# ACCtools/alignasm

Measured on AMD Instinct MI355X. Metric: contigs_per_sec, higher is better.
Workload: dtype int64

## Files before the change

### alignasm_amd/csrc/aasm_kernels.h

```cpp
#pragma once
#include <cstddef>
#include "aasm_dev.h"
#include "../../include/alignasm_amd.h"

namespace aasm {

struct PqK;
struct WS {
    int64_t C, R, R0, S, VT, ET;
    int32_t K, nsl;
    int32_t avg_sidetracks;
    int32_t xcd_map;
    int32_t mw_compact;
    int32_t sort_depth_test;
    const int64_t *rec_off, *in_qs, *in_qe, *in_rs, *in_re, *in_qt, *in_rng_off, *rql, *rqr, *rrl;
    const int32_t *in_chr;
    const uint8_t *in_fwd, *in_mq;
    const char *cs_text;
    const int64_t *cs_off;
    int64_t *rng_rec;
    int64_t rng_stride;
    int32_t *cs_bad;
    int32_t *perm, *dupflag, *np, *pstart;
    int64_t *s_qs, *s_qe, *s_rs, *s_re, *s_qt, *s_rb;
// ... 3047 lines not shown
}

#if defined(AASM_HOST_EMUL)
static int64_t g_k9_stat[64];
#define K9STAT(i, n) (g_k9_stat[i] += (n))
#else
#define K9STAT(i, n) do {} while (0)
#endif
struct SelCtx {
    const WS *w;
    int64_t c, b, N, V, vb, cap;
    int32_t src, dest;
    int32_t *pathA, *pathB, *pathT, *pre2, *stamp;
    Dist *dist2;
    OutElem *cur;
    int64_t *cls;
    int32_t epoch, last_head, last_pos;
    int32_t res_ppos;
    int32_t *out_dst;
    int32_t out_n, out_flushed;
    int32_t pa_base, pa_n;
    int32_t wu, wv, wpv, wvf;
    int32_t cw_pa, cw_n;
    bool err, res_lds;
    int lane;
    char *lds;
    int64_t n_ispr_e, n_ispr_v, n_path_e, n_out_e;
#if defined(AASM_KPROF) && !defined(AASM_HOST_EMUL)
    int64_t kp_t0, kp_acc[8];
#endif
};
#if defined(AASM_KPROF) && !defined(AASM_HOST_EMUL)
#define SPROF(s, i) do { __builtin_amdgcn_s_waitcnt(0); const int64_t t1_ = (int64_t)__builtin_amdgcn_s_memtime(); __builtin_amdgcn_s_waitcnt(0); (s).kp_acc[i] += t1_ - (s).kp_t0; (s).kp_t0 = t1_; } while (0)
#else
#define SPROF(s, i) do {} while (0)
#endif

#define ISPR_MAX_E 192
#define SEL_WIN 64
struct SelLds {
    int32_t pb_buf[2 * SEL_WIN];
    int64_t wq[ISPR_MAX_E];
    int32_t wr[ISPR_MAX_E];
    int8_t tgt[ISPR_MAX_E];
    uint8_t fl[ISPR_MAX_E];
    Dist dist[64];
    int32_t excl[64], u[64], vj[64];
    int8_t pre[64];
    uint8_t reach[64];
    int32_t res[2 * 64];
};
#define AASM_SEL_LDS_BYTES 6656
#define AASM_SELREC_LDS_BYTES 512
static_assert(sizeof(SelLds) <= AASM_SEL_LDS_BYTES, "LDS budget");
static_assert(offsetof(SelLds, wq) == AASM_SELREC_LDS_BYTES, "kb_sel_recover allocates the write buffer alone");
#define ISPR_WIDE 127
struct SelWide { Dist dist[ISPR_WIDE + 1]; int32_t excl[ISPR_WIDE + 2]; int32_t vj[ISPR_WIDE + 1]; uint8_t pre[ISPR_WIDE + 1]; uint8_t reach[ISPR_WIDE + 1]; };
static_assert(offsetof(SelLds, wq) + sizeof(SelWide) <= offsetof(SelLds, res), "the wide DP state must end before the result array");

AASM_DEV void sel_out_flush(SelCtx &s) {
    SelLds *L = (SelLds *)s.lds;
    wave_lds_sync();
    const int32_t n = s.out_n - s.out_flushed;
    for (int32_t t = s.lane; t < 2 * n; t += AASM_WAVE) s.out_dst[2 * s.out_flushed + t] = L->pb_buf[t];
    s.out_flushed = s.out_n;
    wave_lds_sync();
}
AASM_DEV void sel_out_begin(SelCtx &s, int32_t *dst) { s.out_dst = dst; s.out_n = 0; s.out_flushed = 0; }
AASM_DEV void sel_push(SelCtx &s, int32_t u, int32_t v, int32_t pos_v) {
    SelLds *L = (SelLds *)s.lds;
    if (s.out_n >= s.cap) { s.err = true; return; }
    const int32_t slot = s.out_n - s.out_flushed;
    if (s.lane == 0) { L->pb_buf[2 * slot] = u; L->pb_buf[2 * slot + 1] = v; }
    s.out_n++;
    s.last_head = v; s.last_pos = pos_v;
    if (s.out_n - s.out_flushed == SEL_WIN) sel_out_flush(s);
}
#if !defined(AASM_HOST_EMUL)
AASM_DEV void sel_push_lanes(SelCtx &s, int32_t l0, int32_t m, int32_t u, int32_t v) {
    SelLds *L = (SelLds *)s.lds;
    if (s.out_n + m > s.cap) { s.err = true; return; }
    const int32_t slot0 = s.out_n - s.out_flushed, room = SEL_WIN - slot0;
    const int32_t first = m < room ? m : room;
    const int32_t k = s.lane - l0;
    if (k >= 0 && k < first) { L->pb_buf[2 * (slot0 + k)] = u; L->pb_buf[2 * (slot0 + k) + 1] = v; }
    s.out_n += first;
    if (s.out_n - s.out_flushed == SEL_WIN) sel_out_flush(s);
    if (m > first) {
        if (k >= first && k < m) { L->pb_buf[2 * (k - first)] = u; L->pb_buf[2 * (k - first) + 1] = v; }
        s.out_n += m - first;
    }
}
#endif

AASM_DEV int32_t sel_recover(SelCtx &s, int32_t kidx) {
    const WS &w = *s.w;
    const int64_t K = w.K;
    if (kidx < 0 || kidx >= w.kfound[s.c]) return 0;
    const I4 *kcand = w.kcand + 2 * s.c * (3 * K + 1);
    const HNode *nodes = heap_arena(w, s.c);
    int32_t ns = 0;
    int32_t cur = w.klast[s.c * K + kidx];
    while (cur != -1) {
        if (ns >= s.cap) { s.err = true; return -1; }
        const I4 cd = kcand[2 * (int64_t)cur];
        const HNode nd = nodes[cd.x];
        if (s.lane == 0) { s.pathT[2 * ns] = nd.u; s.pathT[2 * ns + 1] = nd.v; }
        ns++;
        cur = cd.y;
    }
    wave_fence();
    sel_out_begin(s, s.pathA);
    int32_t idx = ns - 1, cv = s.src;
    int32_t st_u = -1, st_v = -1;
    if (idx >= 0) { st_u = uni(s.pathT[2 * idx]); st_v = uni(s.pathT[2 * idx + 1]); }
    while (cv != s.dest || idx >= 0) {
        if (s.err) return -1;
        if (idx >= 0 && cv == st_u) {
            sel_push(s, cv, st_v, -1);
            cv = st_v; idx--;
            if (idx >= 0) { st_u = uni(s.pathT[2 * idx]); st_v = uni(s.pathT[2 * idx + 1]); }
        } else {
            const int32_t *rec = w.tnx16 + 16 * (s.vb + cv);
#if defined(AASM_HOST_EMUL)
            for (int t = 0; t < 16; t++) {
                const int32_t nx = rec[t];
                if (nx < 0) { s.err = true; return -1; }
                sel_push(s, cv, nx, -1);
                cv = nx;
                if (s.err || cv == s.dest || (idx >= 0 && cv == st_u)) break;
            }
#else
            const bool in = s.lane < 16;
            const int32_t x = in ? rec[s.lane] : -1;
            const uint64_t stop = wave_ballot(in && (x == s.dest || (idx >= 0 && x == st_u)));
            const uint64_t bad = wave_ballot(in && x < 0);
            const int32_t m = stop ? ffs64(stop) : 16;
            if (bad && ffs64(bad) <= m) { s.err = true; return -1; }
            int32_t from = wave_shfl_up(x, 1, cv);
            if (s.lane == 0) from = cv;
            sel_push_lanes(s, 0, m, from, x);
            cv = wave_bcast(x, m - 1);
#endif
        }
    }
    if (s.err) return -1;
    sel_out_flush(s);
    return s.out_n;
}

#define SETTLE_SCAN_MAX 48
AASM_DEV void sel_classify_edge(const WS &w, int64_t vb, int32_t dest, const int32_t *pathA, int32_t la, int32_t t, int32_t *mark, int32_t ord, int64_t *cls) {
    const int32_t tu = pathA[2 * t], hv = pathA[2 * t + 1];
    const int32_t nvv = (t + 1 < la) ? pathA[2 * t + 3] : -1;
    const int32_t a = w.v_i[vb + hv], b = w.v_j[vb + hv];
    const int32_t pu = w.fwd_pos[vb + tu], pv = w.fwd_pos[vb + hv];
    const int32_t pnv = nvv >= 0 ? w.fwd_pos[vb + nvv] : -1;
    if (hv != dest) {
        atomic_min_i32(&mark[a], ord);
        if (b != a) atomic_min_i32(&mark[b], ord);
    }
    int32_t fl = (a == b) ? 1 : 0;
    const int32_t dpos = pnv - pu;
    if (nvv >= 0 && (dpos == 2 || dpos == 3)) {
        const int64_t *tp = w.tp_ptr + vb + pu;
        const int64_t p0 = tp[0], p1 = tp[1], p2 = tp[2], p3 = (dpos == 3) ? tp[3] : p2;
        if (p3 - p0 <= SETTLE_SCAN_MAX) {
            const bool y_first = pv == pu + 2;
            const int32_t py = y_first ? pu + 1 : pu + 2;
            bool u_nv = false, u_y = false, y_nv = false, y_v = false, v_y = false;
            for (int64_t e = p0; e < p3; e++) {
                const int32_t tg = w.te_pk[e].x;
                const int32_t row = e < p1 ? 0 : e < p2 ? 1 : 2;
                if (row == 0) { u_nv |= tg == pnv; u_y |= tg == py; }
// ... 549 lines not shown
                    const int64_t up = (dd.qry + dd.ref) - (mind.qry + mind.ref), down = (int64_t)mind.anom - dd.anom;
                    int32_t kind = -1;
                    if (ans_idx == -1 || up * ans_down < down * ans_up) { ans_up = up; ans_down = down; ans_idx = i; ans_d = dd; kind = 2; }
                    else if (dist_sel_equal(dd, ans_d)) kind = 3;
                    if (kind >= 0) { if (k.lane == 0) put(n, i, kind); n++; }
                }
            }
        }
    }
    return n;
}
AASM_DEV void kb_sel_plan(const KCtx &k, const WS &w) {
    const int64_t c = k.bid;
    const int32_t n = sel_has_graph(w, c) ? sel_plan_wave(k, w, c, false) : 0;
    if (k.lane == 0) w.nconv[c] = n;
}
AASM_DEV void kb_sel_planfill(const KCtx &k, const WS &w) {
    const int64_t c = k.bid;
    if (!sel_has_graph(w, c)) return;
    const int32_t n = w.nconv[c];
    if (n > SEL_PLAN_KEEP) { sel_plan_wave(k, w, c, true); return; }
    const int32_t N = (int32_t)(w.rec_off[c + 1] - w.rec_off[c]), V = w.ctgV[c];
    const int32_t *keep = w.plan_kk + c * (int64_t)(2 * SEL_PLAN_KEEP);
    const int64_t j0 = w.conv_off[c];
    for (int32_t t = k.lane; t < n; t += AASM_WAVE) {
        const int64_t j = j0 + t;
        w.cv_ctg[j] = (int32_t)c; w.cv_k[j] = keep[2 * t]; w.cv_ord[j] = t; w.cv_kind[j] = keep[2 * t + 1]; w.cv_szr[j] = N + 2; w.cv_szv[j] = V;
    }
}

AASM_DEV void sel_ctx_init(SelCtx &s, const KCtx &k, const WS &w, int64_t c) {
    const int64_t gb = w.rec_off[c];
    s.w = &w; s.c = c; s.b = gb - w.R0; s.N = w.rec_off[c + 1] - gb; s.V = w.ctgV[c]; s.vb = w.voff[c]; s.cap = s.N + 2;
    s.src = (int32_t)(s.V - 2); s.dest = (int32_t)(s.V - 1);
    s.epoch = 0; s.last_head = -1; s.last_pos = -1; s.res_ppos = -1; s.err = false; s.res_lds = false; s.out_dst = nullptr; s.out_n = s.out_flushed = 0;
    s.pa_base = 0; s.pa_n = 0; s.wu = s.wv = s.wpv = s.wvf = 0; s.cls = nullptr;
    s.lane = k.lane; s.lds = k.lds; s.n_ispr_e = s.n_ispr_v = s.n_path_e = s.n_out_e = 0;
    s.cw_pa = -1; s.cw_n = 0;
}
AASM_DEV void sel_flush_counters(const SelCtx &s, const WS &w) {
    if (s.lane == 0) {
        atomic_add(&w.counters[CNT_ISPR_E], s.n_ispr_e); atomic_add(&w.counters[CNT_ISPR_V], s.n_ispr_v);
        atomic_add(&w.counters[CNT_PATH_E], s.n_path_e); atomic_add(&w.counters[CNT_OUT_E], s.n_out_e);
    }
}

AASM_DEV void sel_conv_setup(SelCtx &s, const KCtx &k, const WS &w, int64_t j) {
    sel_ctx_init(s, k, w, w.cv_ctg[j]);
    const int64_t ro = w.cv_roff[j], vo = w.cv_voff[j];
    s.pathA = w.cv_path + 6 * ro; s.pathB = s.pathA + 2 * s.cap; s.pathT = s.pathB + 2 * s.cap;
    s.pre2 = w.cv_pre2 + vo; s.stamp = w.cv_stamp + vo; s.dist2 = w.cv_dist2 + vo;
    s.cur = w.cv_out + ro; s.cls = (int64_t *)s.cur;
}
AASM_DEV void kb_sel_recover(const KCtx &k, const WS &w) {
    const int64_t j = k.bid;
    SelCtx s;
    sel_conv_setup(s, k, w, j);
    const int32_t la = sel_recover(s, w.cv_k[j]);
    if (k.lane == 0) w.cv_la[j] = (la <= 0 || s.err) ? -1 : la;
}
AASM_DEV void kb_sel_classify(const KCtx &k, const WS &w) {
    const int64_t j = k.bid;
    const int32_t la = w.cv_la[j];
    if (la <= 0) return;
    const int64_t c = w.cv_ctg[j], vb = w.voff[c], ro = w.cv_roff[j];
    const int32_t dest = w.ctgV[c] - 1;
    const int64_t cap = (w.rec_off[c + 1] - w.rec_off[c]) + 2;
    (void)cap;
    int32_t *mark = w.mark_time + (w.rec_off[c] - w.R0);
    for (int32_t t = k.tid; t < la; t += k.nthreads) sel_classify_edge(w, vb, dest, w.cv_path + 6 * ro, la, t, mark, w.cv_ord[j], (int64_t *)(w.cv_out + ro));
}
AASM_DEV void kb_sel_convert(const KCtx &k, const WS &w) {
    const int64_t j = k.bid;
    const int64_t c = w.cv_ctg[j];
    SelCtx s;
    sel_conv_setup(s, k, w, j);
#if defined(AASM_KPROF) && !defined(AASM_HOST_EMUL)
    for (int i_ = 0; i_ < 8; i_++) s.kp_acc[i_] = 0;
    __builtin_amdgcn_s_waitcnt(0); s.kp_t0 = (int64_t)__builtin_amdgcn_s_memtime(); __builtin_amdgcn_s_waitcnt(0);
#endif
    int64_t cov = 0;
    int32_t n = 0;
    const int32_t la = w.cv_la[j];
    if (la <= 0) s.err = true;
    else { K9STAT(0, 1); K9STAT(1, la); n = sel_upgrade_emit(s, la, cov); }
    if (k.lane == 0) { w.cv_n[j] = n; w.cv_cov[j] = cov; w.cv_err[j] = s.err ? 1 : 0; }
#if defined(AASM_KPROF) && !defined(AASM_HOST_EMUL)
    if (k.lane == 0 && w.cv_ord[j] == 0) for (int i_ = 0; i_ < 8; i_++) w.prof_sel[c * 8 + i_] = s.kp_acc[i_];
#endif
    (void)c;
    sel_flush_counters(s, w);
}

AASM_DEV void sel_all_append(const KCtx &k, const WS &w, int64_t c, const OutElem *src, int32_t n, const int32_t *mark, int32_t ord) {
    int64_t off = 0, r = 0;
    if (k.lane == 0) { off = (int64_t)atomic_add(&w.counters[CNT_POOL], (int64_t)n); r = (int64_t)atomic_add(&w.counters[CNT_AR], (int64_t)1); }
    off = wave_bcast(off, 0); r = wave_bcast(r, 0);
    if (off + n <= w.pool_cap && r < w.ar_cap) {
        copy_resolved(w.pool + off, src, n, mark, ord, k.lane);
        if (k.lane == 0) { w.ar_ctg[r] = (int32_t)c; w.ar_gen[r] = w.all_gen[c]; w.ar_seq[r] = w.all_seq[c]; w.ar_off[r] = off; w.ar_len[r] = n; }
    } else if (k.lane == 0) {
        atomic_add(&w.counters[CNT_OVF], (int64_t)1);
    }
    if (k.lane == 0) w.all_seq[c] += 1;
    wave_fence();
}

AASM_DEV void kb_sel_final(const KCtx &k, const WS &w) {
    const int64_t c = k.bid;
    const int64_t gb = w.rec_off[c], N = w.rec_off[c + 1] - gb, b = gb - w.R0;
    const bool L0 = (k.lane == 0);
// ... 204 lines not shown
```

### alignasm_amd/csrc/aasm_pipeline.h

```cpp
#pragma once
#include <algorithm>
#include <cstdlib>
#include <cstring>
#include <map>
#include <string>
#include <vector>

#include "../../include/alignasm_amd.h"
#include "aasm_kernels.h"
#include "aasm_enum.h"

namespace aasm {

enum Kern {
#define AASM_PIPELINE_KERNELS(K, KL)                                                                                                  \
    K(KN_CS_RANGES, aasm_k0_cs_ranges, 256, ALL_LANES, kb_cs_ranges)                                                                  \
    KL(KN_SORT, aasm_k1_sort, 256, 1, AASM_SORT_LDS_BYTES, 2, kb_sort)                                                                \
    K(KN_SORT_RANK, aasm_k1_sort_rank, 256, ALL_LANES, kb_sort_rank)                                                                  \
    KL(KN_SORT_FIX, aasm_k1_sort_fix, AASM_WAVE, 1, AASM_SORTFIX_LDS_BYTES, 1, kb_sort_fix)                                           \
    K(KN_GATHER_PARTS, aasm_k1_gather_parts, AASM_WAVE, 1, kb_gather_parts)                                                           \
    K(KN_OV_COUNT, aasm_k2_ov_count, 256, ALL_LANES, kb_ov_count)                                                                     \
    K(KN_OV_MERGE, aasm_k2_ov_merge, 256, ALL_LANES, kb_ov_merge)                                                                     \
    K(KN_VCOUNT, aasm_k2_vcount, 256, ALL_LANES, kb_vcount)                                                                           \
    K(KN_VFILL_REC, aasm_k2_vfill_rec, 256, ALL_LANES, kb_vfill_rec)                                                                  \
    K(KN_VFILL_SLOT, aasm_k2_vfill_slot, 256, ALL_LANES, kb_vfill_slot)                                                               \
    K(KN_NSL, aasm_k4_nsl, 256, ALL_LANES, kb_nsl)                                                                                    \
    K(KN_ROW_COUNT, aasm_k4_row_count, 256, ALL_LANES, kb_row_count)                                                                  \
    K(KN_ROW_FILL, aasm_k4_row_fill, AASM_WAVE, 1, kb_row_fill)                                                                       \
                               \
    KL(KN_GRAPH, aasm_k46_graph, GB_TPB, 1, AASM_GB_LDS_BYTES, 5, kb_graph_build<GB_MAXV, GB_MAXE>)                                   \
                                                     \
    KL(KN_GRAPH_L, aasm_k46_graph_l, GB_TPB, 1, AASM_GB_LDS_BYTES_T(GB_MAXV_L, GB_MAXE_L), 2, kb_graph_build<GB_MAXV_L, GB_MAXE_L>)   \
    K(KN_REV_FILL, aasm_k6_rev_fill, 256, ALL_LANES, kb_rev_fill)                                                                     \
    KL(KN_REV_FILL_W, aasm_k6_rev_fill_w, AASM_WAVE, 1, AASM_REVF_LDS_BYTES, 8, kb_rev_fill_w)                                        \
                    \
    KL(KN_REV_FILL_ORD, aasm_k6_rev_fill_ord, AASM_WAVE, 1, AASM_REVO_LDS_BYTES, 2, kb_rev_fill_ord)                                  \
    KL(KN_REV_FILL_ORD_S, aasm_k6_rev_fill_ord_s, AASM_WAVE, 1, AASM_REVO_LDS_BYTES_V(REV_ORD_MIDV), 6, kb_rev_fill_ord)              \
    KL(KN_SORT_ROWS_REV, aasm_k6_rev_place, AASM_WAVE, 1, AASM_REVP_LDS_BYTES, 4, kb_rev_place)                                       \
    K(KN_REV_HDR, aasm_k6_rev_hdr, 256, ALL_LANES, kb_rev_hdr)                                                                        \
    KL(KN_REV_SWEEP, aasm_k6_rev_sweep, AASM_WAVE, 1, AASM_REV_LDS_BYTES, 8, kb_rev_sweep<AASM_WAVE>)                                 \
    KL(KN_FWD_SWEEP, aasm_k5_fwd_sweep, AASM_WAVE, 1, AASM_FWD_LDS_BYTES, 8, kb_fwd_sweep<AASM_WAVE>)                                 \
    KL(KN_REV_SWEEP_G, aasm_k6_rev_sweep_g, AASM_WAVE, 1, (AASM_WAVE / AASM_SWEEP_G) * AASM_REV_LDS_BYTES, 4, kb_rev_sweep<AASM_SWEEP_G>) \
    KL(KN_FWD_SWEEP_G, aasm_k5_fwd_sweep_g, AASM_WAVE, 1, (AASM_WAVE / AASM_SWEEP_G) * AASM_FWD_LDS_BYTES, 4, kb_fwd_sweep<AASM_SWEEP_G>) \
    K(KN_CHILDREN, aasm_k7_children, 256, ALL_LANES, kb_children)                                                                     \
    K(KN_HEAP_CAP, aasm_k7_heap_cap, 256, ALL_LANES, kb_heap_cap)                                                                     \
    KL(KN_SIDETRACK_W, aasm_k7_sidetrack_w, AASM_WAVE, 1, AASM_SIDE_LDS_BYTES, 8, kb_sidetrack_w)                                     \
    K(KN_HEAP_HDR, aasm_k7_heap_hdr, 256, ALL_LANES, kb_heap_hdr)                                                                     \
    KL(KN_HEAP, aasm_k7_heap, AASM_WAVE, 1, AASM_HEAP_LDS_BYTES, 5, kb_heap<false, HEAP_RING_1W, HEAP_QN_1W>)                         \
    KL(KN_HEAP_MW, aasm_k7_heap_mw, AASM_WAVE * 4, 1, AASM_MW_LDS_BYTES(4), 4, kb_heap_mw)                                            \
    KL(KN_HEAP_MW8, aasm_k7_heap_mw8, AASM_WAVE * 8, 1, AASM_MW_LDS_BYTES(8), 4, kb_heap_mw)                                          \
    KL(KN_HEAP_MW16, aasm_k7_heap_mw16, AASM_WAVE * 16, 1, AASM_MW_LDS_BYTES(16), 4, kb_heap_mw)                                      \
    K(KN_MW_RANK, aasm_k7_mw_rank, 256, ALL_LANES, kb_mw_rank)                                                                        \
                                    \
    KL(KN_ENUM, aasm_k8_enum, AASM_WAVE, 1, AASM_EMUL_OR(AASM_ENUM_LDS_BYTES, AASM_ENUM2_LDS_BYTES), 4,                               \
       AASM_EMUL_OR(kb_enum_heap, kb_enum_lsm<64>))                                                                                   \
    KL(KN_ENUM_S, aasm_k8_enum_s, AASM_WAVE, 1, AASM_EMUL_OR(AASM_ENUM_LDS_BYTES, AASM_ENUM2_LDS_BYTES_F(EQ_FSMALL)), 5,              \
       AASM_EMUL_OR(kb_enum_heap, kb_enum_lsm<EQ_FSMALL>))                                                                            \
    KL(KN_ENUM_HEAP, aasm_k8_enum_heap, AASM_WAVE, 1, AASM_ENUM_LDS_BYTES, 2, kb_enum_heap)                                           \
    KL(KN_SELECT, aasm_k9_select, AASM_WAVE, 1, AASM_SEL_LDS_BYTES, 5, kb_select)                                                     \
    K(KN_GATHER_OUT, aasm_k9_gather_out, AASM_WAVE, 1, kb_gather_out)                                                                 \
    K(KN_TOPO_COUNT, aasm_k9_topo_count, 256, ALL_LANES, kb_topo_count)                                                               \
    K(KN_TOPO_FILL, aasm_k9_topo_fill, AASM_WAVE, 1, kb_topo_fill)                                                                    \
    K(KN_SEL_PLAN, aasm_k9_sel_plan, AASM_WAVE, 1, kb_sel_plan)                                                                       \
    K(KN_SEL_PLANFILL, aasm_k9_sel_planfill, AASM_WAVE, 1, kb_sel_planfill)                                                           \
    KL(KN_SEL_RECOVER, aasm_k9_sel_recover, AASM_WAVE, 1, AASM_SELREC_LDS_BYTES, 8, kb_sel_recover)                                   \
    K(KN_SEL_CLASSIFY, aasm_k9_sel_classify, 256, ALL_LANES, kb_sel_classify)                                                         \
    KL(KN_SEL_CONVERT, aasm_k9_sel_convert, AASM_WAVE, 1, AASM_SEL_LDS_BYTES, 5, kb_sel_convert)                                      \
    K(KN_SEL_FINAL, aasm_k9_sel_final, AASM_WAVE, 1, kb_sel_final)                                                                    \
            \
    KL(KN_CHAIN, aasm_k67_chain, AASM_WAVE * CHAIN_WAVES, CHAIN_WAVES, AASM_CHAIN_LDS_BYTES, 5, kb_chain<true>)                       \
                 \
    KL(KN_CHAIN3, aasm_k67_chain3, AASM_WAVE * (CHAIN_WAVES - 1), CHAIN_WAVES - 1, AASM_CHAIN_LDS_BYTES, 5, kb_chain<false>)          \
    K(KN_K7_PREP, aasm_k7_prep, 256, ALL_LANES, kb_k7_prep)                                                                           \
    K(KN_TNX, aasm_k9_tnx, 256, ALL_LANES, kb_tnx)                                                                                    \
    K(KN_TNX16, aasm_k9_tnx16, 256, ALL_LANES, kb_tnx16)                                                                              \
                                                                  \
    KL(KN_TNX16_WG, aasm_k9_tnx16_wg, TNX_TPB, 1, AASM_TNXWG_LDS_BYTES, 4, kb_tnx16_wg)
    AASM_PIPELINE_KERNELS(AASM_ROW_ID, AASM_ROW_ID)
};
constexpr int kern_block[] = {AASM_PIPELINE_KERNELS(AASM_ROW_BLOCK, AASM_ROW_BLOCK)};

AASM_DEV void run_kernel_body(int kn, const KCtx &k, const WS &w) {
    switch (kn) {
#define K(id, sym, block, lanes, ...) case id: __VA_ARGS__(k, w); break;
#define KL(id, sym, block, lanes, lds, waves, ...) case id: __VA_ARGS__(k, w); break;
        AASM_PIPELINE_KERNELS(K, KL)
#undef K
#undef KL
    }
}

template <class B> void launch(B &be, int kn, int64_t nblocks, const WS &w) { be.launch(kn, nblocks, kern_block[kn], w); }

static inline int64_t cdiv(int64_t a, int64_t b) { return (a + b - 1) / b; }
#ifndef AASM_CHAIN_ORD_MAX
#define AASM_CHAIN_ORD_MAX 1024
#endif
#define AASM_CHAIN_SMALL_BATCH 1536

#ifndef AASM_GROUPED_MIN
#define AASM_GROUPED_MIN 2560
#endif
struct PipelineSizes { int64_t C = 0, R = 0, S = 0, VT = 0, ET = 0, HT = 0, bad_record = -1; };

struct Hooks {
    bool seq_select, enum_heap, enum_small, grid_order, graph_launches, chain_half, launch_failure, wrap_devices, dirty_scan, chain_own_queue;
    int32_t heap_mw, chain, chain_test, root_ring, sort_depth;
    int32_t mw;
    int64_t range_limit;
};
static inline Hooks decode_hooks(const aasm_opts &o) {
    const int32_t h0 = o.reserved[0], h2 = o.reserved[2], ch = h0 & AASM_H0_CHAIN_MASK;
    Hooks h;
    h.seq_select = h0 & AASM_H0_SEQ_SELECT; h.enum_heap = h0 & AASM_H0_ENUM_HEAP; h.enum_small = h0 & AASM_H0_ENUM_SMALL;
    h.grid_order = h0 & AASM_H0_GRID_ORDER; h.graph_launches = h0 & AASM_H0_GRAPH_LAUNCHES; h.chain_half = ch == AASM_H0_CHAIN_HALF;
    h.heap_mw = (h0 & AASM_H0_HEAP_MW_ALL) ? 1 : (h0 & AASM_H0_HEAP_MW_NONE) ? 2 : 0;
    h.chain = ch == AASM_H0_CHAIN_ALL ? 1 : ch == AASM_H0_CHAIN_NONE ? 2 : 0;
    h.mw = (h0 & AASM_H0_MW_MASK) >> AASM_H0_MW_SHIFT; h.range_limit = o.reserved[1];
    h.launch_failure = h2 & AASM_H2_LAUNCH_FAILURE; h.wrap_devices = h2 & AASM_H2_WRAP_DEVICES; h.dirty_scan = h2 & AASM_H2_DIRTY_SCAN;
    h.chain_test = (h2 & AASM_H2_CHAIN_DONE_LOST) ? 2 : (h2 & AASM_H2_CHAIN_HDR_LOST) ? 1 : 0; h.chain_own_queue = h2 & AASM_H2_CHAIN_OWN_QUEUE;
    h.root_ring = (h2 & AASM_H2_SMALL_ROOT_RING) ? 4 : 0; h.sort_depth = (h2 & AASM_H2_SORT_DEPTH_MASK) >> AASM_H2_SORT_DEPTH_SHIFT;
    return h;
}

struct FormSizes { int64_t C, R, K, VT, ET, MAXV, NCHAIN, HTM, NMW, MAXN; };
struct Forms {
    bool grouped, dense, mw_ranked;
    int rev_fill, chain, mw_kern, enum_kern;
};
static inline Forms choose_forms(const FormSizes &s, const Hooks &h, bool host_emulation) {
    Forms f;
    f.dense = s.ET > 6 * s.VT;
    f.grouped = !f.dense && s.C >= AASM_GROUPED_MIN;
    f.rev_fill = f.dense && s.MAXV <= REV_ORD_MAXV ? (s.MAXV <= REV_ORD_MIDV ? KN_REV_FILL_ORD_S : KN_REV_FILL_ORD) : f.dense ? KN_REV_FILL_W : KN_REV_FILL;
    f.chain = !h.chain_own_queue && s.NCHAIN <= AASM_CHAIN_ORD_MAX ? KN_CHAIN : KN_CHAIN3;
    const int mw_waves = (h.mw == 4 || h.mw == 8 || h.mw == 16) ? h.mw : s.NMW * 16 <= 6144 ? 16 : s.NMW * 8 <= 6144 ? 8 : 4;
    f.mw_kern = mw_waves == 16 ? KN_HEAP_MW16 : mw_waves == 8 ? KN_HEAP_MW8 : KN_HEAP_MW;
    f.mw_ranked = h.mw != AASM_H0_MW_INPUT_ORDER && s.NMW >= 2 && s.NMW <= 32768;
    const bool enum_heap = host_emulation || h.enum_heap || s.MAXN > AASM_ENUM_MAX_N;
    f.enum_kern = enum_heap ? KN_ENUM_HEAP : ((s.C > 14 * 256 && s.C <= 20 * 256 && s.K > 21) || h.enum_small) ? KN_ENUM_S : KN_ENUM;
    return f;
}

template <class B>
int run_pipeline(B &be, const aasm_batch_in &in, const aasm_opts &opts, WS &w, PipelineSizes &sz) {
    std::memset(&w, 0, sizeof(w));
    const int64_t C = in.n_contigs;
    int64_t rr[2];
    be.read_i64s({in.ctg_rec_off, in.ctg_rec_off + C}, rr);
    const int64_t R0 = rr[0], R1 = rr[1];
    const int64_t R = R1 - R0;
    w.C = C; w.R = R; w.R0 = R0;
    w.K = opts.max_paths > 0 ? opts.max_paths : 10000;
    w.nsl = opts.non_skip_linkable ? 1 : 0;
    const Hooks h = decode_hooks(opts);
    w.xcd_map = h.grid_order ? 0 : 1; w.sort_depth_test = h.sort_depth;
    w.chain_mode = h.chain; w.chain_test = h.chain_test; w.chain_rn = h.root_ring;
    w.chain_ord = h.chain_own_queue ? 0 : 1;
    w.chain_all = (!h.chain_half && C <= AASM_CHAIN_SMALL_BATCH) ? 1 : 0;
    w.chain_minN = (int32_t)std::min<int64_t>(std::max<int64_t>(2048, 4 * (R / std::max<int64_t>(C, 1))), INT32_MAX);
    if (h.chain_half) w.chain_minN = (int32_t)std::min<int64_t>(std::max<int64_t>(1, cdiv(R, std::max<int64_t>(C, 1))), INT32_MAX);
    w.rec_off = in.ctg_rec_off; w.in_qs = in.qry_str; w.in_qe = in.qry_end; w.in_rs = in.ref_str; w.in_re = in.ref_end;
    w.in_qt = in.qry_total; w.in_chr = in.ref_chr; w.in_fwd = in.aln_fwd; w.in_mq = in.map_qul;
    w.in_rng_off = in.rec_rng_off; w.rql = in.rng_qry_l; w.rqr = in.rng_qry_r; w.rrl = in.rng_ref_l; w.rng_stride = 1;
    sz.C = C; sz.R = R;
    if (C <= 0 || R <= 0) return AASM_E_INVAL;

#define A(field, type, n, name) w.field = (type *)be.alloc(name, sizeof(type) * (size_t)((n) > 0 ? (n) : 1))
#define AZ(field, type, n, name) do { A(field, type, n, name); be.zero_alloc(w.field, sizeof(type) * (size_t)((n) > 0 ? (n) : 1)); } while (0)
#define CHECK_ALLOC() do { if (be.oom()) return AASM_E_NOMEM; if (be.failed()) return AASM_E_HIP; } while (0)

    AZ(status, int32_t, C, "status");
    AZ(prof_heap, int64_t, C * 8, "prof_heap"); AZ(prof_sel, int64_t, C * 8, "prof_sel"); AZ(prof_gb, int64_t, C * 8, "prof_gb");
    AZ(counters, int64_t, CNT_N, "counters");
    AZ(dupflag, int32_t, C, "dupflag");
    AZ(main_len, int32_t, C, "main_len"); AZ(alt_len, int32_t, C, "alt_len"); AZ(all_gen, int32_t, C, "all_gen"); AZ(all_seq, int32_t, C, "all_seq");
    AZ(kfound, int32_t, C, "kfound"); AZ(anom_dest, int32_t, C, "anom_dest"); AZ(h_cnt, int32_t, C, "h_cnt");
    AZ(nconv, int32_t, C, "nconv");

    if (!in.rng_qry_l && in.cs_text && in.rec_cs_off) {
        if (R > INT32_MAX) return AASM_E_INVAL;
        int64_t gg[2];
        be.read_i64s({in.rec_rng_off + R0, in.rec_rng_off + R1}, gg);
        const int64_t G0 = gg[0], G1 = gg[1];
        be.phase_begin(AASM_PH_CS);
        w.cs_text = in.cs_text; w.cs_off = in.rec_cs_off;
        A(rng_rec, int64_t, 4 * (G1 - G0), "rng_rec"); A(cs_bad, int32_t, 2, "cs_bad");
        CHECK_ALLOC();
        w.rng_rec -= 4 * G0;
        be.zero(w.cs_bad, 8);
        launch(be, KN_CS_RANGES, cdiv(R, 256), w);
        be.phase_end(AASM_PH_CS);
        const int32_t badv = (int32_t)(uint32_t)(uint64_t)be.read_i64((const int64_t *)w.cs_bad);
        if (badv != 0) { sz.bad_record = R0 + ((int64_t)badv + INT32_MAX); return AASM_E_PARSE; }
        w.rql = w.rng_rec; w.rqr = w.rng_rec + 1; w.rrl = w.rng_rec + 2; w.rng_stride = 4;
    } else if (!in.rng_qry_l) return AASM_E_INVAL;

    be.phase_begin(AASM_PH_SORT);
    A(perm, int32_t, R, "perm"); A(np, int32_t, C, "np"); A(pstart, int32_t, R + C, "pstart");
    A(s_qs, int64_t, R, "s_qs"); A(s_qe, int64_t, R, "s_qe"); A(s_rs, int64_t, R, "s_rs"); A(s_re, int64_t, R, "s_re");
    A(s_qt, int64_t, R, "s_qt"); A(s_rb, int64_t, R, "s_rb"); A(s_rn, int32_t, R, "s_rn"); A(s_chr, int32_t, R, "s_chr");
    A(s_orig, int32_t, R, "s_orig"); A(s_ctg, int32_t, R, "s_ctg"); A(s_pid, int32_t, R, "s_pid"); A(s_fl, uint8_t, R, "s_fl");
    CHECK_ALLOC();
    if (h.launch_failure) be.launch(KN_SORT, C, 4096, w);
    launch(be, KN_SORT, C, w);
    launch(be, KN_SORT_RANK, cdiv(R, 256), w);
    launch(be, KN_SORT_FIX, C, w);
    launch(be, KN_GATHER_PARTS, C, w);
    be.phase_end(AASM_PH_SORT);

    be.phase_begin(AASM_PH_PAIRS);
    A(ov_cnt, int32_t, R, "ov_cnt"); A(ov_off, int64_t, R + 1, "ov_off");
    CHECK_ALLOC();
    launch(be, KN_OV_COUNT, cdiv(R, 256), w);
    be.scan_i32(w.ov_cnt, R, w.ov_off);
    const int64_t S = be.read_i64(w.ov_off + R);
    w.S = S; sz.S = S;
    A(ov_rec, int32_t, S, "ov_rec"); A(ov_vid, int32_t, S, "ov_vid"); A(ov_rank, int64_t, S + 1, "ov_rank");
    A(ov_peq, int64_t, S, "ov_peq"); A(ov_per, int64_t, S, "ov_per"); A(ov_stq, int64_t, S, "ov_stq"); A(ov_str, int64_t, S, "ov_str");
    A(ov_ok, uint8_t, S, "ov_ok");
    CHECK_ALLOC();
    if (S > 0) launch(be, KN_OV_MERGE, cdiv(S, 256), w);
    be.scan_u8(w.ov_ok, S, w.ov_rank);
    A(ctgV, int32_t, C, "ctgV"); A(voff, int64_t, C + 1, "voff");
    CHECK_ALLOC();
    launch(be, KN_VCOUNT, cdiv(C, 256), w);
    be.scan_i32(w.ctgV, C, w.voff);
    const int64_t VT = be.read_i64(w.voff + C);
    w.VT = VT; sz.VT = VT;
    A(v_i, int32_t, VT, "v_i"); A(v_j, int32_t, VT, "v_j"); A(v_ctg, int32_t, VT, "v_ctg"); A(v_slot, int64_t, VT, "v_slot");
    CHECK_ALLOC();
    launch(be, KN_VFILL_REC, cdiv(R, 256), w);
    if (S > 0) launch(be, KN_VFILL_SLOT, cdiv(S, 256), w);
    be.phase_end(AASM_PH_PAIRS);

    A(cur_out, OutElem, R, "cur_out"); A(main_out, OutElem, R, "main_out"); A(alt_out, OutElem, R, "alt_out");
    A(main_off, int64_t, C + 1, "main_off"); A(alt_off, int64_t, C + 1, "alt_off");
    w.pool_cap = R + 1024; w.ar_cap = C + R / 4 + 1024;
    A(pool, OutElem, w.pool_cap, "pool");
    A(ar_ctg, int32_t, w.ar_cap, "ar_ctg"); A(ar_gen, int32_t, w.ar_cap, "ar_gen"); A(ar_seq, int32_t, w.ar_cap, "ar_seq");
    A(ar_len, int32_t, w.ar_cap, "ar_len"); A(ar_off, int64_t, w.ar_cap, "ar_off");
    CHECK_ALLOC();

    if (VT > 0) {
        be.phase_begin(AASM_PH_EDGES);
        if (w.nsl) {
            A(dis_end, int32_t, R, "dis_end"); AZ(next_cnt, int32_t, R, "next_cnt");
            CHECK_ALLOC();
            launch(be, KN_NSL, cdiv(R, 256), w);
        }
        A(deg, int32_t, VT, "deg"); A(rowptr, int64_t, VT + 1, "csr_rowptr");
        A(hcap_cnt, int32_t, C, "hcap_cnt"); A(hoff, int64_t, C + 1, "hoff");
        A(mw_flag, int32_t, C, "mw_flag"); A(mw_lg, int32_t, C, "mw_lg"); A(mw_cap, int32_t, C, "mw_cap"); A(mw_off, int64_t, C + 1, "mw_off"); A(mw_list, int32_t, C, "mw_list"); A(mw_sorted, int32_t, C, "mw_sorted"); A(mw_key, int32_t, C, "mw_key");
        A(chain_flag, int32_t, C, "chain_flag"); A(chain_list, int32_t, C, "chain_list"); A(gb_flag, int32_t, C, "gb_flag");
        w.gb_off = h.graph_launches ? 1 : 0;
        w.mw_mode = h.heap_mw;
        w.mw_compact = opts.keep_debug ? 1 : 0;
        CHECK_ALLOC();
        launch(be, KN_ROW_COUNT, cdiv(VT, 256), w);
        be.scan_i32(w.deg, VT, w.rowptr);
        launch(be, KN_HEAP_CAP, cdiv(C, 256), w);
        be.scan_i32_pair(w.hcap_cnt, w.hoff, w.mw_cap, w.mw_off, C);
        int64_t et_mv[12];
        be.read_i64s({w.rowptr + VT, w.counters + CNT_MAXV, w.hoff + C, w.mw_off + C, w.counters + CNT_MW, w.counters + CNT_MAXN, w.counters + CNT_CHAIN, w.counters + CNT_GB_S, w.counters + CNT_GB_L, w.counters + CNT_GB_REST}, et_mv);
        const int64_t ET = et_mv[0], MAXV = et_mv[1];
        const int64_t GB_S = et_mv[7], GB_L = et_mv[8], GB_REST = et_mv[9];
        const int64_t hh[4] = {et_mv[2], et_mv[3], et_mv[4], et_mv[5]};
        const int64_t NCHAIN = et_mv[6];
        const int64_t HT = hh[0], HTM = hh[1], NMW = HTM > 0 ? hh[2] : 0;
        const Forms f = choose_forms({C, R, w.K, VT, ET, MAXV, NCHAIN, HTM, NMW, hh[3]}, h, B::host_emulation);
        w.chain_ord = f.chain == KN_CHAIN ? 1 : 0;
        w.ET = ET; sz.ET = ET;
        A(e_col, int32_t, ET, "csr_col"); A(e_wq, int64_t, ET, "csr_w_qry"); A(e_wr, int32_t, ET, "csr_w_ref"); A(e_fl, uint8_t, ET, "csr_w_flags");
        A(rptr, int64_t, VT + 1, "rptr"); A(r_pk, I4, ET, "r_pk");
        A(rvh, I4, 3 * VT, "rvh"); A(fvh, I4, 2 * VT, "fvh");
        A(sp_d, Dist, VT, "sp_d"); A(sp_best, int32_t, VT, "sp_best"); A(cnt_tmp, int32_t, VT, "cnt_tmp"); A(cnt_tmp2, int32_t, VT, "cnt_tmp2"); A(an, int32_t, VT, "an");
        if (NCHAIN > 0) { A(pend, int32_t, VT, "pend"); A(cq, int32_t, VT, "cq"); A(bfsq, I4, VT, "bfsq"); }
        w.indeg = nullptr;
        if (GB_REST > 0) { AZ(indeg, int32_t, VT, "indeg"); AZ(rcur, int32_t, VT, "rcur"); }
        CHECK_ALLOC();
        if (GB_S > 0) launch(be, KN_GRAPH, C, w);
        if (GB_L > 0) launch(be, KN_GRAPH_L, C, w);
        if (GB_REST == 0) {
            be.phase_end(AASM_PH_EDGES);
            be.phase_begin(AASM_PH_REVCSR);
            be.phase_end(AASM_PH_REVCSR);
        } else {
        launch(be, KN_ROW_FILL, cdiv(VT, AASM_WAVE), w);
        be.phase_end(AASM_PH_EDGES);

        be.phase_begin(AASM_PH_REVCSR);
        A(r_e, int32_t, ET, "r_e"); A(tmp_pk, I4, ET, "tmp_pk");
        CHECK_ALLOC();
        be.scan_i32(w.indeg, VT, w.rptr);
        if (f.rev_fill == KN_REV_FILL_ORD_S || f.rev_fill == KN_REV_FILL_ORD) launch(be, f.rev_fill, C, w);
        else {
            if (f.rev_fill == KN_REV_FILL_W) launch(be, KN_REV_FILL_W, cdiv(VT, AASM_WAVE), w);
            else launch(be, KN_REV_FILL, cdiv(VT, 256), w);
            launch(be, KN_SORT_ROWS_REV, cdiv(VT, AASM_WAVE), w);
        }
        launch(be, KN_REV_HDR, cdiv(VT, 256), w);
        be.phase_end(AASM_PH_REVCSR);
        }

        A(rev_order, int32_t, VT, "rev_order"); A(fwd_order, int32_t, VT, "fwd_order"); A(fwd_pos, int32_t, VT, "fwd_pos");
        A(tp_deg, int32_t, VT, "tp_deg"); A(tp_vj, int32_t, VT, "tp_vj"); A(tp_ptr, int64_t, VT + 1, "tp_ptr");
        A(te_pk, I4, ET, "te_pk");
        CHECK_ALLOC();
        const int64_t sweep_n = AASM_WAVE / AASM_SWEEP_G;
        auto side_work = [&]() {
            be.fork();
            be.use_side(true);
            be.phase_begin(AASM_PH_FWD);
            if (f.grouped) launch(be, KN_FWD_SWEEP_G, cdiv(C, sweep_n), w);
            else launch(be, KN_FWD_SWEEP, C, w);
            be.phase_end(AASM_PH_FWD);
            be.phase_begin(AASM_PH_TOPO);
            launch(be, KN_TOPO_COUNT, cdiv(VT, 256), w);
            be.scan_i32(w.tp_deg, VT, w.tp_ptr);
            launch(be, KN_TOPO_FILL, cdiv(VT, AASM_WAVE), w);
            be.phase_end(AASM_PH_TOPO);
            be.use_side(false);
        };
        side_work();
        A(ccnt, int32_t, VT, "ccnt"); A(cval, int32_t, ET, "cval");
        A(st_cost, Dist, ET, "st_cost"); A(st_n, int32_t, VT, "st_n"); A(vhdr, I4, VT, "vhdr"); A(vhdr2, I4, VT, "vhdr2"); A(cinfo, I4, ET, "cinfo"); A(tnx, I4, VT, "tnx"); A(tnx16, int32_t, 16 * VT, "tnx16");
        sz.HT = HT;
        w.avg_sidetracks = (int32_t)std::min<int64_t>((ET - VT + C) / (C > 0 ? C : 1), INT32_MAX);
        A(hnodes, HNode, HT, "hnodes"); A(h_root, int32_t, VT, "h_root"); A(bq, int32_t, VT, "bq");
        A(hprov, HNode, HTM, "hprov");
        A(mw_order, int32_t, VT, "mw_order"); A(mw_rs, int32_t, VT, "mw_rs"); A(mw_fb, int32_t, VT, "mw_fb"); A(mw_rsv, int32_t, VT, "mw_rsv"); A(mw_used, int32_t, VT, "mw_used");
        CHECK_ALLOC();
        be.fill_ff(w.h_root, sizeof(int32_t) * (size_t)VT);
        be.fill_ff(w.bq, sizeof(int32_t) * (size_t)VT);
        if (NCHAIN > 0) {
            be.fill_ff(w.vhdr, sizeof(I4) * (size_t)VT);
            be.fill_ff(w.vhdr2, sizeof(I4) * (size_t)VT);
            be.fork2();
            be.use_side2(true);
            be.phase_begin(AASM_PH_CHAIN);
            if (f.chain == KN_CHAIN) launch(be, KN_CHAIN, NCHAIN, w);
            else launch(be, KN_CHAIN3, NCHAIN, w);
            be.phase_end(AASM_PH_CHAIN);
            be.use_side2(false);
        }
        if (NCHAIN < C) {
        be.phase_begin(AASM_PH_SPTREE);
        if (f.grouped) launch(be, KN_REV_SWEEP_G, cdiv(C, sweep_n), w);
        else launch(be, KN_REV_SWEEP, C, w);
        be.phase_end(AASM_PH_SPTREE);

        be.fork_again();
        be.use_side(true);
        if (GB_S + GB_L > 0) launch(be, KN_TNX16_WG, C, w);
        if (GB_REST > 0) {
            launch(be, KN_TNX, cdiv(VT, 256), w);
            launch(be, KN_TNX16, cdiv(VT, 256), w);
        }
        be.use_side(false);
        be.phase_begin(AASM_PH_HEAP_PREP);
        if (f.dense) {
            launch(be, KN_CHILDREN, cdiv(VT, 256), w);
            launch(be, KN_SIDETRACK_W, cdiv(VT, AASM_WAVE), w);
            launch(be, KN_HEAP_HDR, cdiv(VT, 256), w);
        } else launch(be, KN_K7_PREP, cdiv(VT, 256), w);
        be.phase_end(AASM_PH_HEAP_PREP);
        be.join();
        be.phase_begin(AASM_PH_HEAP);
        launch(be, KN_HEAP, C, w);
        w.mw_n = (int32_t)NMW; w.mw_base = -1;
        if (HTM > 0) {
            if (f.mw_ranked) {
                launch(be, KN_MW_RANK, cdiv(NMW, 256), w);
                w.mw_base = 0;
                { const int32_t xm = w.xcd_map; w.xcd_map = 0; launch(be, f.mw_kern, NMW, w); w.xcd_map = xm; }
                w.mw_base = -1;
            } else launch(be, f.mw_kern, C, w);
        }
        be.phase_end(AASM_PH_HEAP);
        }
        be.join2();

        const int64_t K = w.K;
        A(kd, Dist, C * K, "kd"); A(klast, int32_t, C * K, "klast");
        w.pq_stride = f.enum_kern == KN_ENUM_HEAP ? 3 * K + 1 : enum_stride(K);
        A(kcand, I4, 2 * C * (3 * K + 1), "kcand"); A(pq, PqK, C * w.pq_stride, "pq");
        CHECK_ALLOC();
        be.phase_begin(AASM_PH_ENUM);
        launch(be, f.enum_kern, C, w);
        be.phase_end(AASM_PH_ENUM);
    }

    be.join();
    A(mark_time, int32_t, R, "mark_time");
    A(conv_off, int64_t, C + 1, "conv_off"); A(plan_kk, int32_t, C * 2 * SEL_PLAN_KEEP, "plan_kk");
    CHECK_ALLOC();
    be.fill_byte(w.mark_time, 0x7F, sizeof(int32_t) * (size_t)R);
    bool sequential = h.seq_select;
    int64_t NCONV = 0, SR = 0, SV = 0;
    bool nm_ready = false;
    int64_t nm[2] = {0, 0};
    if (!sequential) {
        be.phase_begin(AASM_PH_MISC);
        if (VT > 0) launch(be, KN_SEL_PLAN, C, w);
        be.scan_i32(w.nconv, C, w.conv_off);
        NCONV = be.read_i64(w.conv_off + C);
        w.NCONV = NCONV;
        if (NCONV > 0) {
            A(cv_ctg, int32_t, NCONV, "cv_ctg"); A(cv_k, int32_t, NCONV, "cv_k"); A(cv_ord, int32_t, NCONV, "cv_ord"); A(cv_kind, int32_t, NCONV, "cv_kind");
            A(cv_szr, int32_t, NCONV, "cv_szr"); A(cv_szv, int32_t, NCONV, "cv_szv"); A(cv_roff, int64_t, NCONV + 1, "cv_roff"); A(cv_voff, int64_t, NCONV + 1, "cv_voff");
            AZ(cv_n, int32_t, NCONV, "cv_n"); AZ(cv_err, int32_t, NCONV, "cv_err"); AZ(cv_cov, int64_t, NCONV, "cv_cov"); A(cv_la, int32_t, NCONV, "cv_la");
            CHECK_ALLOC();
            launch(be, KN_SEL_PLANFILL, C, w);
            be.scan_i32_pair(w.cv_szr, w.cv_roff, w.cv_szv, w.cv_voff, NCONV);
            int64_t sv[2];
            be.read_i64s({w.cv_roff + NCONV, w.cv_voff + NCONV}, sv);
            SR = sv[0]; SV = sv[1];
            const int64_t bytes = SR * (24 + (int64_t)sizeof(OutElem)) + SV * ((int64_t)sizeof(Dist) + 8);
            if (bytes > ((int64_t)24 << 30)) sequential = true;
        }
        be.phase_end(AASM_PH_MISC);
    }
    if (!sequential) {
        if (NCONV > 0) {
            A(cv_path, int32_t, 6 * SR, "cv_path"); A(cv_out, OutElem, SR, "cv_out");
            A(cv_dist2, Dist, SV, "cv_dist2"); A(cv_pre2, int32_t, SV, "cv_pre2"); AZ(cv_stamp, int32_t, SV, "cv_stamp");
            CHECK_ALLOC();
            be.phase_begin(AASM_PH_SELECT);
            launch(be, KN_SEL_RECOVER, NCONV, w);
            launch(be, KN_SEL_CLASSIFY, NCONV, w);
            launch(be, KN_SEL_CONVERT, NCONV, w);
            be.phase_end(AASM_PH_SELECT);
        }
        be.phase_begin(AASM_PH_FINAL);
        launch(be, KN_SEL_FINAL, C, w);
        be.scan_i32_pair(w.main_len, w.main_off, w.alt_len, w.alt_off, C);
        int64_t np2[4];
        be.read_i64s({w.counters + CNT_POOL, w.counters + CNT_AR, w.main_off + C, w.alt_off + C}, np2);
        const int64_t need_pool = np2[0], need_ar = np2[1];
        nm_ready = true; nm[0] = np2[2]; nm[1] = np2[3];
        if (need_pool > w.pool_cap || need_ar > w.ar_cap) {
            w.pool_cap = need_pool + 16; w.ar_cap = need_ar + 16;
            A(pool, OutElem, w.pool_cap, "pool");
            A(ar_ctg, int32_t, w.ar_cap, "ar_ctg"); A(ar_gen, int32_t, w.ar_cap, "ar_gen"); A(ar_seq, int32_t, w.ar_cap, "ar_seq");
            A(ar_len, int32_t, w.ar_cap, "ar_len"); A(ar_off, int64_t, w.ar_cap, "ar_off");
            CHECK_ALLOC();
            be.zero(w.all_seq, sizeof(int32_t) * (size_t)C);
            be.zero(w.counters + CNT_POOL, sizeof(int64_t)); be.zero(w.counters + CNT_AR, sizeof(int64_t)); be.zero(w.counters + CNT_OVF, sizeof(int64_t));
            launch(be, KN_SEL_FINAL, C, w);
            nm_ready = false;
        }
        be.phase_end(AASM_PH_FINAL);
    } else {
        A(pathA, int32_t, 2 * (R + 2 * C), "pathA"); A(pathB, int32_t, 2 * (R + 2 * C), "pathB"); A(pathT, int32_t, 2 * (R + 2 * C), "pathT");
        A(pre2, int32_t, VT, "pre2"); AZ(stamp, int32_t, VT, "stamp"); A(dist2, Dist, VT, "dist2");
        CHECK_ALLOC();
        be.phase_begin(AASM_PH_SELECT);
        launch(be, KN_SELECT, C, w);
        be.phase_end(AASM_PH_SELECT);
        int64_t np2[2];
        be.read_i64s({w.counters + CNT_POOL, w.counters + CNT_AR}, np2);
        const int64_t need_pool = np2[0], need_ar = np2[1];
        if (need_pool > w.pool_cap || need_ar > w.ar_cap) {
            w.pool_cap = need_pool + 16; w.ar_cap = need_ar + 16;
            A(pool, OutElem, w.pool_cap, "pool");
            A(ar_ctg, int32_t, w.ar_cap, "ar_ctg"); A(ar_gen, int32_t, w.ar_cap, "ar_gen"); A(ar_seq, int32_t, w.ar_cap, "ar_seq");
            A(ar_len, int32_t, w.ar_cap, "ar_len"); A(ar_off, int64_t, w.ar_cap, "ar_off");
            CHECK_ALLOC();
            be.zero(w.stamp, sizeof(int32_t) * (size_t)(VT > 0 ? VT : 1));
            be.fill_byte(w.mark_time, 0x7F, sizeof(int32_t) * (size_t)R);
            be.zero(w.all_gen, sizeof(int32_t) * (size_t)C); be.zero(w.all_seq, sizeof(int32_t) * (size_t)C);
            be.zero(w.counters + CNT_POOL, sizeof(int64_t)); be.zero(w.counters + CNT_AR, sizeof(int64_t));
            be.zero(w.counters + CNT_CONVERTED, sizeof(int64_t)); be.zero(w.counters + CNT_OVF, sizeof(int64_t));
            be.zero(w.counters + CNT_ISPR_E, sizeof(int64_t)); be.zero(w.counters + CNT_ISPR_V, sizeof(int64_t));
            be.zero(w.counters + CNT_PATH_E, sizeof(int64_t)); be.zero(w.counters + CNT_OUT_E, sizeof(int64_t));
            be.phase_begin(AASM_PH_MISC);
            launch(be, KN_SELECT, C, w);
            be.phase_end(AASM_PH_MISC);
        }
    }

    be.phase_begin(AASM_PH_GATHER);
    if (!nm_ready) {
        be.scan_i32_pair(w.main_len, w.main_off, w.alt_len, w.alt_off, C);
        be.read_i64s({w.main_off + C, w.alt_off + C}, nm);
    }
    const int64_t NM = nm[0], NA = nm[1];
    A(main_c, OutElem, NM, "main_c"); A(alt_c, OutElem, NA, "alt_c");
    CHECK_ALLOC();
    launch(be, KN_GATHER_OUT, C, w);
    be.phase_end(AASM_PH_GATHER);
#undef A
#undef AZ
#undef CHECK_ALLOC
    return AASM_OK;
}

template <class B>
int fetch_results(B &be, const WS &w, const PipelineSizes &sz, aasm_batch_out *out) {
    std::memset(out, 0, sizeof(*out));
    const int64_t C = w.C;
    out->n_contigs = C;
    out->main_off = (int64_t *)calloc(C + 1, 8);
    out->alt_off = (int64_t *)calloc(C + 1, 8);
    out->all_path_off = (int64_t *)calloc(C + 1, 8);
    out->ctg_status = (int32_t *)calloc(C + 1, 4);
    be.d2h(out->main_off, w.main_off, (C + 1) * 8);
    be.d2h(out->alt_off, w.alt_off, (C + 1) * 8);
    be.d2h(out->ctg_status, w.status, C * 4);
    const int64_t NM = out->main_off[C], NA = out->alt_off[C];
// ... 151 lines not shown
```

Baseline: 449,500.

## Recover selected paths from an LDS shortest-path tree instead of precomputed tnx16 records

```diff
diff --git a/alignasm_amd/csrc/aasm_kernels.h b/alignasm_amd/csrc/aasm_kernels.h
--- a/alignasm_amd/csrc/aasm_kernels.h
+++ b/alignasm_amd/csrc/aasm_kernels.h
@@ -3123,6 +3123,13 @@
 };
 #define AASM_SEL_LDS_BYTES 6656
 #define AASM_SELREC_LDS_BYTES 512
+#ifndef AASM_RECOVER_LDS
+#define AASM_RECOVER_LDS 1
+#endif
+#define SEL_TREE_END 0xFFFF
+#define AASM_SELREC_TREE_LDS_BYTES(maxv) (AASM_SELREC_LDS_BYTES + 2 * (maxv))
+struct SelTree { uint16_t nx[GB_MAXV_L]; };
+static_assert(GB_MAXV_L < SEL_TREE_END && AASM_SELREC_LDS_BYTES + sizeof(SelTree) == AASM_SELREC_TREE_LDS_BYTES(GB_MAXV_L), "LDS budget");
 static_assert(sizeof(SelLds) <= AASM_SEL_LDS_BYTES, "LDS budget");
 static_assert(offsetof(SelLds, wq) == AASM_SELREC_LDS_BYTES, "kb_sel_recover allocates the write buffer alone");
 #define ISPR_WIDE 127
@@ -3164,7 +3171,29 @@
 }
 #endif
 
-AASM_DEV int32_t sel_recover(SelCtx &s, int32_t kidx) {
+AASM_DEV bool sel_tree_class(const WS &w, int64_t c) { return AASM_RECOVER_LDS && in_graph_class(w, c) && !in_chain_class(w, c); }
+#define SEL_TREE_LOADS (GB_MAXV / AASM_WAVE)
+AASM_DEV void sel_tree_load(const SelCtx &s, SelTree *T) {
+    const int32_t *best = s.w->sp_best + s.vb;
+    const int32_t V = (int32_t)s.V;
+#if defined(AASM_HOST_EMUL)
+    for (int32_t v = 0; v < V; v++) { const int32_t b = best[v]; T->nx[v] = (uint16_t)((b >= 0 && b < V) ? b : SEL_TREE_END); }
+#else
+    for (int32_t v0 = 0; v0 < V; v0 += SEL_TREE_LOADS * AASM_WAVE) {
+        int32_t b[SEL_TREE_LOADS];
+        AASM_UNROLL
+        for (int i = 0; i < SEL_TREE_LOADS; i++) { const int32_t v = v0 + i * AASM_WAVE + s.lane; b[i] = v < V ? best[v] : -1; }
+        AASM_UNROLL
+        for (int i = 0; i < SEL_TREE_LOADS; i++) {
+            const int32_t v = v0 + i * AASM_WAVE + s.lane;
+            if (v < V) T->nx[v] = (uint16_t)((b[i] >= 0 && b[i] < V) ? b[i] : SEL_TREE_END);
+        }
+    }
+    wave_lds_sync();
+#endif
+}
+
+AASM_DEV int32_t sel_recover(SelCtx &s, int32_t kidx, const SelTree *tree = nullptr) {
     const WS &w = *s.w;
     const int64_t K = w.K;
     if (kidx < 0 || kidx >= w.kfound[s.c]) return 0;
@@ -3191,6 +3220,37 @@
             sel_push(s, cv, st_v, -1);
             cv = st_v; idx--;
             if (idx >= 0) { st_u = uni(s.pathT[2 * idx]); st_v = uni(s.pathT[2 * idx + 1]); }
+        } else if (tree) {
+#if defined(AASM_HOST_EMUL)
+            for (int t = 0; t < 64; t++) {
+                const int32_t nx = tree->nx[cv];
+                if (nx == SEL_TREE_END) { s.err = true; return -1; }
+                sel_push(s, cv, nx, -1);
+                cv = nx;
+                if (s.err || cv == s.dest || (idx >= 0 && cv == st_u)) break;
+            }
+#else
+            int32_t x = cv, head = -1, n = 0;
+            uint64_t stop = 0, bad = 0;
+            do {
+                AASM_UNROLL
+                for (int t = 0; t < 16; t++) {
+                    const int32_t nx = tree->nx[x == SEL_TREE_END ? 0 : x];
+                    x = x == SEL_TREE_END ? SEL_TREE_END : nx;
+                    if (s.lane == n + t) head = x;
+                }
+                n += 16;
+                const bool in = s.lane < n;
+                stop = wave_ballot(in && (head == s.dest || (idx >= 0 && head == st_u)));
+                bad = wave_ballot(in && head == SEL_TREE_END);
+            } while (!(stop | bad) && n < AASM_WAVE);
+            const int32_t m = stop ? ffs64(stop) : n;
+            if (bad && ffs64(bad) <= m) { s.err = true; return -1; }
+            int32_t from = wave_shfl_up(head, 1, cv);
+            if (s.lane == 0) from = cv;
+            sel_push_lanes(s, 0, m, from, head);
+            cv = wave_bcast(head, m - 1);
+#endif
         } else {
             const int32_t *rec = w.tnx16 + 16 * (s.vb + cv);
 #if defined(AASM_HOST_EMUL)
@@ -3846,11 +3906,19 @@
     s.pre2 = w.cv_pre2 + vo; s.stamp = w.cv_stamp + vo; s.dist2 = w.cv_dist2 + vo;
     s.cur = w.cv_out + ro; s.cls = (int64_t *)s.cur;
 }
+template <int MAXV>
 AASM_DEV void kb_sel_recover(const KCtx &k, const WS &w) {
     const int64_t j = k.bid;
     SelCtx s;
     sel_conv_setup(s, k, w, j);
-    const int32_t la = sel_recover(s, w.cv_k[j]);
+    const SelTree *tree = nullptr;
+    if (sel_tree_class(w, s.c)) {
+        if (s.V > MAXV) { if (k.lane == 0) w.cv_la[j] = -1; return; }
+        SelTree *T = (SelTree *)(k.lds + AASM_SELREC_LDS_BYTES);
+        sel_tree_load(s, T);
+        tree = T;
+    }
+    const int32_t la = sel_recover(s, w.cv_k[j], tree);
     if (k.lane == 0) w.cv_la[j] = (la <= 0 || s.err) ? -1 : la;
 }
 AASM_DEV void kb_sel_classify(const KCtx &k, const WS &w) {
diff --git a/alignasm_amd/csrc/aasm_pipeline.h b/alignasm_amd/csrc/aasm_pipeline.h
--- a/alignasm_amd/csrc/aasm_pipeline.h
+++ b/alignasm_amd/csrc/aasm_pipeline.h
@@ -63,7 +63,7 @@
     K(KN_TOPO_FILL, aasm_k9_topo_fill, AASM_WAVE, 1, kb_topo_fill)                                                                    \
     K(KN_SEL_PLAN, aasm_k9_sel_plan, AASM_WAVE, 1, kb_sel_plan)                                                                       \
     K(KN_SEL_PLANFILL, aasm_k9_sel_planfill, AASM_WAVE, 1, kb_sel_planfill)                                                           \
-    KL(KN_SEL_RECOVER, aasm_k9_sel_recover, AASM_WAVE, 1, AASM_SELREC_LDS_BYTES, 8, kb_sel_recover)                                   \
+    KL(KN_SEL_RECOVER, aasm_k9_sel_recover, AASM_WAVE, 1, AASM_SELREC_LDS_BYTES, 8, kb_sel_recover<0>)                                \
     K(KN_SEL_CLASSIFY, aasm_k9_sel_classify, 256, ALL_LANES, kb_sel_classify)                                                         \
     KL(KN_SEL_CONVERT, aasm_k9_sel_convert, AASM_WAVE, 1, AASM_SEL_LDS_BYTES, 5, kb_sel_convert)                                      \
     K(KN_SEL_FINAL, aasm_k9_sel_final, AASM_WAVE, 1, kb_sel_final)                                                                    \
@@ -75,7 +75,10 @@
     K(KN_TNX, aasm_k9_tnx, 256, ALL_LANES, kb_tnx)                                                                                    \
     K(KN_TNX16, aasm_k9_tnx16, 256, ALL_LANES, kb_tnx16)                                                                              \
                                                                   \
-    KL(KN_TNX16_WG, aasm_k9_tnx16_wg, TNX_TPB, 1, AASM_TNXWG_LDS_BYTES, 4, kb_tnx16_wg)
+    KL(KN_TNX16_WG, aasm_k9_tnx16_wg, TNX_TPB, 1, AASM_TNXWG_LDS_BYTES, 4, kb_tnx16_wg)                                               \
+                 \
+    KL(KN_SEL_RECOVER_S, aasm_k9_sel_recover_s, AASM_WAVE, 1, AASM_SELREC_TREE_LDS_BYTES(GB_MAXV), 8, kb_sel_recover<GB_MAXV>)        \
+    KL(KN_SEL_RECOVER_L, aasm_k9_sel_recover_l, AASM_WAVE, 1, AASM_SELREC_TREE_LDS_BYTES(GB_MAXV_L), 6, kb_sel_recover<GB_MAXV_L>)
     AASM_PIPELINE_KERNELS(AASM_ROW_ID, AASM_ROW_ID)
 };
 constexpr int kern_block[] = {AASM_PIPELINE_KERNELS(AASM_ROW_BLOCK, AASM_ROW_BLOCK)};
@@ -123,10 +126,11 @@
     return h;
 }
 
-struct FormSizes { int64_t C, R, K, VT, ET, MAXV, NCHAIN, HTM, NMW, MAXN; };
+struct FormSizes { int64_t C, R, K, VT, ET, MAXV, NCHAIN, HTM, NMW, MAXN, GB_S, GB_L; };
 struct Forms {
     bool grouped, dense, mw_ranked;
     int rev_fill, chain, mw_kern, enum_kern;
+    int recover;
 };
 static inline Forms choose_forms(const FormSizes &s, const Hooks &h, bool host_emulation) {
     Forms f;
@@ -139,6 +143,7 @@
     f.mw_ranked = h.mw != AASM_H0_MW_INPUT_ORDER && s.NMW >= 2 && s.NMW <= 32768;
     const bool enum_heap = host_emulation || h.enum_heap || s.MAXN > AASM_ENUM_MAX_N;
     f.enum_kern = enum_heap ? KN_ENUM_HEAP : ((s.C > 14 * 256 && s.C <= 20 * 256 && s.K > 21) || h.enum_small) ? KN_ENUM_S : KN_ENUM;
+    f.recover = (!AASM_RECOVER_LDS || s.GB_S + s.GB_L == 0) ? KN_SEL_RECOVER : s.GB_L == 0 ? KN_SEL_RECOVER_S : KN_SEL_RECOVER_L;
     return f;
 }
 
@@ -242,6 +247,8 @@
     A(ar_len, int32_t, w.ar_cap, "ar_len"); A(ar_off, int64_t, w.ar_cap, "ar_off");
     CHECK_ALLOC();
 
+    int recover_kern = KN_SEL_RECOVER;
+    bool wg_records_missing = false;
     if (VT > 0) {
         be.phase_begin(AASM_PH_EDGES);
         if (w.nsl) {
@@ -268,7 +275,8 @@
         const int64_t hh[4] = {et_mv[2], et_mv[3], et_mv[4], et_mv[5]};
         const int64_t NCHAIN = et_mv[6];
         const int64_t HT = hh[0], HTM = hh[1], NMW = HTM > 0 ? hh[2] : 0;
-        const Forms f = choose_forms({C, R, w.K, VT, ET, MAXV, NCHAIN, HTM, NMW, hh[3]}, h, B::host_emulation);
+        const Forms f = choose_forms({C, R, w.K, VT, ET, MAXV, NCHAIN, HTM, NMW, hh[3], GB_S, GB_L}, h, B::host_emulation);
+        recover_kern = f.recover;
         w.chain_ord = f.chain == KN_CHAIN ? 1 : 0;
         w.ET = ET; sz.ET = ET;
         A(e_col, int32_t, ET, "csr_col"); A(e_wq, int64_t, ET, "csr_w_qry"); A(e_wr, int32_t, ET, "csr_w_ref"); A(e_fl, uint8_t, ET, "csr_w_flags");
@@ -324,7 +332,10 @@
         };
         side_work();
         A(ccnt, int32_t, VT, "ccnt"); A(cval, int32_t, ET, "cval");
-        A(st_cost, Dist, ET, "st_cost"); A(st_n, int32_t, VT, "st_n"); A(vhdr, I4, VT, "vhdr"); A(vhdr2, I4, VT, "vhdr2"); A(cinfo, I4, ET, "cinfo"); A(tnx, I4, VT, "tnx"); A(tnx16, int32_t, 16 * VT, "tnx16");
+        A(st_cost, Dist, ET, "st_cost"); A(st_n, int32_t, VT, "st_n"); A(vhdr, I4, VT, "vhdr"); A(vhdr2, I4, VT, "vhdr2"); A(cinfo, I4, ET, "cinfo");
+        const bool wg_records = GB_S + GB_L > 0 && (!AASM_RECOVER_LDS || opts.keep_debug);
+        wg_records_missing = GB_S + GB_L > 0 && !wg_records;
+        if (!AASM_RECOVER_LDS || NCHAIN > 0 || GB_REST > 0 || opts.keep_debug) { A(tnx, I4, VT, "tnx"); A(tnx16, int32_t, 16 * VT, "tnx16"); }
         sz.HT = HT;
         w.avg_sidetracks = (int32_t)std::min<int64_t>((ET - VT + C) / (C > 0 ? C : 1), INT32_MAX);
         A(hnodes, HNode, HT, "hnodes"); A(h_root, int32_t, VT, "h_root"); A(bq, int32_t, VT, "bq");
@@ -350,14 +361,16 @@
         else launch(be, KN_REV_SWEEP, C, w);
         be.phase_end(AASM_PH_SPTREE);
 
-        be.fork_again();
-        be.use_side(true);
-        if (GB_S + GB_L > 0) launch(be, KN_TNX16_WG, C, w);
-        if (GB_REST > 0) {
-            launch(be, KN_TNX, cdiv(VT, 256), w);
-            launch(be, KN_TNX16, cdiv(VT, 256), w);
-        }
-        be.use_side(false);
+        if (wg_records || GB_REST > 0) {
+            be.fork_again();
+            be.use_side(true);
+            if (wg_records) launch(be, KN_TNX16_WG, C, w);
+            if (GB_REST > 0) {
+                launch(be, KN_TNX, cdiv(VT, 256), w);
+                launch(be, KN_TNX16, cdiv(VT, 256), w);
+            }
+            be.use_side(false);
+        }
         be.phase_begin(AASM_PH_HEAP_PREP);
         if (f.dense) {
             launch(be, KN_CHILDREN, cdiv(VT, 256), w);
@@ -427,7 +440,7 @@
             A(cv_dist2, Dist, SV, "cv_dist2"); A(cv_pre2, int32_t, SV, "cv_pre2"); AZ(cv_stamp, int32_t, SV, "cv_stamp");
             CHECK_ALLOC();
             be.phase_begin(AASM_PH_SELECT);
-            launch(be, KN_SEL_RECOVER, NCONV, w);
+            launch(be, recover_kern, NCONV, w);
             launch(be, KN_SEL_CLASSIFY, NCONV, w);
             launch(be, KN_SEL_CONVERT, NCONV, w);
             be.phase_end(AASM_PH_SELECT);
@@ -454,8 +467,10 @@
     } else {
         A(pathA, int32_t, 2 * (R + 2 * C), "pathA"); A(pathB, int32_t, 2 * (R + 2 * C), "pathB"); A(pathT, int32_t, 2 * (R + 2 * C), "pathT");
         A(pre2, int32_t, VT, "pre2"); AZ(stamp, int32_t, VT, "stamp"); A(dist2, Dist, VT, "dist2");
+        if (wg_records_missing && !w.tnx16) A(tnx16, int32_t, 16 * VT, "tnx16");
         CHECK_ALLOC();
         be.phase_begin(AASM_PH_SELECT);
+        if (wg_records_missing) launch(be, KN_TNX16_WG, C, w);
         launch(be, KN_SELECT, C, w);
         be.phase_end(AASM_PH_SELECT);
         int64_t np2[2];
```

Result: no change. 452,800 (median of 6 runs) (+0.7%).
